# CEED/Laghos

Hardware: AMD Instinct MI355X
Metric: Mdofs×steps/s on 3D Sedov -pa (Q3/Q2) (higher is better)
Workload: dtype f64; 1 GPU; 3D Sedov -p 1 -m cube01_hex -rs 4 -ok 3 -ot 2 -pa (32^3 elements, E0/2^dim = 0.125); transport=none (one rank), elements=32768, h1_dofs=2738019, l2_dofs=884736, quad_points_per_element=216, rk_stages_executed=1300, ode=RK4, parallelism=elements1x1x1, zones_per_gpu=32x32x32

## Files before the change

laghos_amd/csrc/lgh_qpoint.hpp:

```cpp
#pragma once
#include "lgh_common.hpp"
#include "lgh_smallmat.hpp"

namespace lgh
{

enum { QMODE_UPDATE = 0, QMODE_SETUP = 1, QMODE_IE = 2, QMODE_KE = 3 };

struct QArgs
{
   int NE, N;
   const double *B, *G, *Bl, *W;
   const int *map;
   const double *x, *v, *e;
   const double *gamma;
   const double *rho0DetJ0w_in;
   const double *Jac0inv_in;
   const double *Jac0inv_soa;
   const double *Jac0inv_e;
   double *Jac0inv_soa_out;
   double *stressJinvT;
   double *Jac0inv_out, *rho0DetJ0w_out, *massD_out;
   const double *rho0_q;
   double *partials;
   unsigned int *ticket;
   double *result;
   double h0, h1order, cfl;
   int visc, vort;
   double *force_e;
   double *erhs_q;
   int q_swz;
   const int *zorder;
   double tiny_grad;
};

__device__ __forceinline__ double smooth_step_01(double x, double eps)
{
   const double y = (x + eps) / (2.0 * eps);
   if (y < 0.0) { return 0.0; }
   if (y > 1.0) { return 1.0; }
   return (3.0 - 2.0 * y) * y * y;
}

template <int DIM, bool VISC = true>
__device__ __forceinline__ double qpoint_body(const QArgs &a, const int e, const size_t eq,
                                              const double weight, const double *J, const double *dV,
                                              const double e_val, const size_t plane,
                                              const double *J0i, const double rho0DetJ0w, double &ftv, double *sjw)
{
   constexpr int DIM2 = DIM * DIM;
   double Jinv[DIM2], stress[DIM2], sgrad_v[DIM2], stressJiT[DIM2];
   const double gamma = a.gamma[e];
   const double inv_weight = 1. / weight;
   const double detJ = sm::det<DIM>(J);
   sm::inverse<DIM>(J, detJ, Jinv);
   const double R = inv_weight * rho0DetJ0w / detJ;
   const double E = fmax(0.0, e_val);
   const double P = (gamma - 1.0) * R * E;
   const double S = sm::fsqrt(gamma * (gamma - 1.0) * E);
#pragma unroll
   for (int k = 0; k < DIM2; k++) { stress[k] = 0.0; }
#pragma unroll
   for (int d = 0; d < DIM; d++) { stress[d * DIM + d] = -P; }
   double visc_coeff = 0.0;
   double s_dot_g;
   if (VISC && a.visc)
   {
      sm::matmul<DIM>(dV, Jinv, sgrad_v);
      double vorticity_coeff = 1.0;
      if (a.vort)
      {
         const double grad_norm = sm::fnorm<DIM>(sgrad_v);
         const double div_v = fabs(sm::trace<DIM>(sgrad_v));
         vorticity_coeff = (grad_norm > 0.0) ? div_v / grad_norm : 1.0;
      }
      sm::symmetrize<DIM>(sgrad_v);
      double mu, compr_dir[DIM], Jpi[DIM2], ph_dir[DIM];
      bool shortcut = false;
      if (DIM == 3 && a.tiny_grad >= 0.0)
      {
         double m = 0.0;
#pragma unroll
         for (int k = 0; k < DIM2; k++) { m = fmax(m, fabs(sgrad_v[k])); }
         shortcut = __all(m <= a.tiny_grad ? 1 : 0) != 0;
      }
      if (shortcut)
      {
         mu = sm::trace<DIM>(sgrad_v) / 3;
#pragma unroll
         for (int d = 0; d < DIM; d++) { compr_dir[d] = (d == 0) ? 1.0 : 0.0; }
      }
      else { sm::min_eigenpair<DIM>(sgrad_v, mu, compr_dir); }
      sm::matvec<DIM>(J0i, compr_dir, Jpi);
      sm::matvec<DIM>(J, Jpi, ph_dir);
      const double ph_dir_nl2 = sm::norml2<DIM>(ph_dir);
      const double compr_dir_nl2 = sm::norml2<DIM>(compr_dir);
      const double H = a.h0 * ph_dir_nl2 / compr_dir_nl2;
      visc_coeff = 2.0 * R * H * H * fabs(mu);
      const double eps = 1e-12;
      visc_coeff += 0.5 * R * H * S * vorticity_coeff * (1.0 - smooth_step_01(mu - 2.0 * eps, eps));
#pragma unroll
      for (int k = 0; k < DIM2; k++) { stress[k] += visc_coeff * sgrad_v[k]; }
      s_dot_g = 0.0;
#pragma unroll
      for (int k = 0; k < DIM2; k++) { s_dot_g += stress[k] * sgrad_v[k]; }
   }
   else
   {
      double divv = 0.0;
#pragma unroll
      for (int i = 0; i < DIM; i++)
#pragma unroll
         for (int d = 0; d < DIM; d++) { divv += dV[i + DIM * d] * Jinv[d + DIM * i]; }
      s_dot_g = -P * divv;
   }
   const double sv = sm::min_singular<DIM>(J);
   const double h_min = sv / a.h1order;
   const double ih_min = 1. / h_min;
   const double irho_ih_min_sq = ih_min * ih_min / R;
   const double idt = S * ih_min + 2.5 * visc_coeff * irho_ih_min_sq;
   double dt_cand = INFINITY;
   if (detJ < 0.0) { dt_cand = 0.0; }
   else if (idt > 0.0) { dt_cand = a.cfl / idt; }
   sm::matmul_abt<DIM>(stress, Jinv, stressJiT);
   const double wd = weight * detJ;
   ftv = s_dot_g * wd;
#pragma unroll
   for (int vd = 0; vd < DIM; vd++)
#pragma unroll
      for (int gd = 0; gd < DIM; gd++)
      {
         const double sv_ = stressJiT[vd + gd * DIM] * wd;
         sjw[gd + vd * DIM] = sv_;
         if (a.stressJinvT) { a.stressJinvT[eq + plane * (gd + vd * DIM)] = sv_; }
      }
   return dt_cand;
}

template <int DIM, int D, int Q, int L, int NEB, int NFMAX, int MODE, int PPT = 1>
__global__ void __launch_bounds__((DIM == 3 ? Q * Q * Q : Q * Q) * NEB / PPT)
qpoint_kernel(const QArgs a)
{
   constexpr int ND = (DIM == 3) ? D * D * D : D * D;
   constexpr int NQ = (DIM == 3) ? Q * Q * Q : Q * Q;
   constexpr int NL = (DIM == 3) ? L * L * L : L * L;
   constexpr int NTE = NQ / PPT;
   static_assert(PPT == 1 || (PPT == 2 && DIM == 3 && MODE == QMODE_UPDATE && Q % 2 == 0), "two points per thread: 3D update only");
   constexpr bool HOIST = (NQ * NEB <= 256) && PPT == 1;
   constexpr bool NEED_X = (MODE == QMODE_UPDATE || MODE == QMODE_SETUP);
   constexpr bool NEED_V = (MODE == QMODE_UPDATE || MODE == QMODE_KE);
   constexpr bool NEED_E = (MODE != QMODE_KE);
   constexpr int NFIELD = (NEED_X ? DIM : 0) + (NEED_V ? DIM : 0);
   constexpr int NF = (NFIELD == 0) ? 1 : (NFMAX < NFIELD ? NFMAX : NFIELD);
   static_assert(PPT == 1 || NF == NFIELD, "two points per thread: all fields in one LDS pass");
   constexpr int SU = NF * ND;
   constexpr int SXs = (DIM == 3) ? 2 * NF * D * D * Q : 2 * NF * D * Q;
   constexpr int SYs = (DIM == 3) ? 3 * NF * D * Q * Q : 0;
   constexpr int SEs = NL + ((DIM == 3) ? (L * L * Q + L * Q * Q) : (L * Q));
   constexpr int PER0 = SU + SXs + SYs + SEs + 1;
   constexpr int FTN = NQ + ((DIM == 3) ? L * Q * Q : 0);
   constexpr int FNEED3 = 9 * NQ + 9 * D * Q * Q + FTN, FNEED1 = 3 * NQ + 3 * D * Q * Q + FTN;
   constexpr int AVAIL = SU + SXs + SYs + ((DIM == 3) ? L * L * L : L * L);
   constexpr int CPR = (DIM == 3 && MODE == QMODE_UPDATE) ? ((AVAIL >= FNEED3) ? 3 : 1) : 0;
   constexpr int GROW = (CPR == 1 && AVAIL < FNEED1) ? FNEED1 - AVAIL : 0;
   constexpr int PER = PER0 + GROW;
   __shared__ double smem[NEB * PER];
   __shared__ double sB[Q * D], sG[Q * D], sBl[Q * L];
   __shared__ double red[16];

   const int tid = threadIdx.x;
   const int lt = tid % NTE, eb = tid / NTE;
   const int tx = lt % Q, ty = (lt / Q) % Q, tz = lt / (Q * Q);
   const int e = blockIdx.x * NEB + eb;
   const bool active = (e < a.NE);
   const int ec = active ? e : a.NE - 1;
   double *sU = smem + eb * PER;
   double *sX = sU + SU;
   double *sY = sX + SXs;
   double *sE = sY + SYs + GROW;
   double *sE1 = sE + NL;
   double *sE2 = sE1 + ((DIM == 3) ? L * L * Q : 0);

   const size_t eq = (size_t)ec * NQ + lt;

   for (int i = tid; i < Q * D; i += NTE * NEB) { sB[i] = a.B[i]; sG[i] = a.G[i]; }
   for (int i = tid; i < Q * L; i += NTE * NEB) { sBl[i] = a.Bl[i]; }
// ... 631 lines not shown
```

laghos_amd/csrc/lgh_qrows.hpp:

```cpp
#pragma once
#include "lgh_qpoint.hpp"

namespace lgh
{

template <int D, int Q, int L> struct QRows
{
   static constexpr int ND = D * D * D, NQ = Q * Q * Q, NL = L * L * L, NF = 6;
   static constexpr int SU = NF * ND;
   static constexpr int SX = NF * Q * D * D;
   static constexpr int SFS = 9 * NQ + NQ;
   static constexpr int R1 = (SU + 2 * SX > SFS) ? SU + 2 * SX : SFS;
   static constexpr int SY = 3 * NF * Q * Q * D;
   static constexpr int SE = NL + L * L * Q + L * Q * Q;
   static constexpr int ST = 2 * Q * D + Q * L;
   static constexpr int TOTAL = R1 + SY + SE + ST;
};

template <int NIN, int NOUT>
__device__ __forceinline__ void row_fwd(const double *__restrict__ T, const double (&in)[NIN], double (&out)[NOUT])
{
#pragma unroll
   for (int q = 0; q < NOUT; q++)
   {
      double s = T[q * NIN] * in[0];
#pragma unroll
      for (int d = 1; d < NIN; d++) { s = fma(T[q * NIN + d], in[d], s); }
      out[q] = s;
   }
}
template <int NIN, int NOUT>
__device__ __forceinline__ void row_bwd(const double *__restrict__ T, const double (&in)[NIN], double (&out)[NOUT])
{
#pragma unroll
   for (int d = 0; d < NOUT; d++)
   {
      double s = T[d] * in[0];
#pragma unroll
      for (int q = 1; q < NIN; q++) { s = fma(T[q * NOUT + d], in[q], s); }
      out[d] = s;
   }
}
template <int N> __device__ __forceinline__ void row_load(const double *__restrict__ p, double (&v)[N])
{
#pragma unroll
   for (int i = 0; i < N; i++) { v[i] = p[i]; }
}

constexpr int kQTraceRec = 16;
template <int D, int Q, int L, int MINW, bool TRACE = false, bool J0C = false>
__global__ void __launch_bounds__(Q *Q *Q, MINW)
qrows_kernel(const QArgs a, unsigned long long *trace = nullptr)
{
   unsigned long long tstamp[12];
#define LGH_QSTAMP(K_) do { if (TRACE) { tstamp[K_] = wall_clock64(); } } while (0)
   LGH_QSTAMP(0);
   using S = QRows<D, Q, L>;
   constexpr int ND = S::ND, NQ = S::NQ, NL = S::NL, NF = S::NF, NT = NQ;
   constexpr int DD = D * D, QQ = Q * Q;
   __shared__ __attribute__((aligned(16))) double smem[S::TOTAL];
   double *const sR1 = smem;
   double *const sU = sR1;
   double *const sX = sR1 + S::SU;
   double *const sF = sR1;
   double *const sS = sR1 + 9 * NQ;
   double *const sW = sR1;
   double *const sY = smem + S::R1;
   double *const sA = sY;
   double *const sTB = sY + S::SY;
   double *const sTG = sTB + Q * D;
   double *const sTL = sTG + Q * D;
   double *const sE = sTL + Q * L;
   double *const sE1 = sE + NL;
   double *const sE2 = sE1 + L * L * Q;

   const int lt = threadIdx.x;
   const int tx = lt % Q, ty = (lt / Q) % Q, tz = lt / QQ;
   int e = blockIdx.x;
   if (a.q_swz < 0) { e = xcd_swizzle(blockIdx.x, gridDim.x); }
   else if (a.q_swz > 0)
   {
      const int R = 1 << a.q_swz, span = 8 * R, b = blockIdx.x;
      if (b < (int)(gridDim.x / span) * span) { e = (b / span) * span + (b & 7) * R + ((b >> 3) & (R - 1)); }
   }
   if (a.zorder) { e = __builtin_amdgcn_readfirstlane(a.zorder[min(e, a.NE - 1)]); }
   const size_t eq = (size_t)e * NQ + lt;
   const size_t plane = (size_t)a.NE * NQ;

   for (int i = lt; i < Q * D; i += NT)
   {
      const int q = i / D, d = i - q * D;
      sTB[i] = a.B[q + Q * d];
      sTG[i] = a.G[q + Q * d];
   }
   for (int i = lt; i < Q * L; i += NT)
   {
      const int q = i / L, l = i - q * L;
      sTL[i] = a.Bl[q + Q * l];
   }
   for (int i = lt; i < 3 * ND; i += NT)
   {
      const int c = i / ND, d = i - c * ND;
      const size_t n = (size_t)c * a.N + a.map[(size_t)e * ND + d];
      sU[i] = a.x[n];
      sU[i + 3 * ND] = a.v[n];
   }
   for (int i = lt; i < NL; i += NT) { sE[i] = a.e[(size_t)e * NL + i]; }
   double J0i[9];
   if (J0C)
   {
#pragma unroll
      for (int k = 0; k < 9; k++) { J0i[k] = uniform_f64(a.Jac0inv_e[(size_t)9 * e + k]); }
   }
   else
   {
#pragma unroll
      for (int k = 0; k < 9; k++) { J0i[k] = a.Jac0inv_soa[eq + plane * k]; }
   }
   const double rdw = a.rho0DetJ0w_in[eq];
   const double weight = a.W[lt];
   LGH_QSTAMP(1);
   __syncthreads();
   LGH_QSTAMP(2);

   for (int i = lt; i < 2 * NF * DD; i += NT)
   {
      const int which = i / (NF * DD), r = i - which * (NF * DD);
      const double *T = sTB + which * (Q * D);
      double u[D], o[Q];
      row_load<D>(sU + D * r, u);
      row_fwd<D, Q>(T, u, o);
      const int f = r / DD, zy = r - f * DD;
      double *dst = sX + which * S::SX + f * (Q * DD) + zy;
#pragma unroll
      for (int q = 0; q < Q; q++) { dst[q * DD] = o[q]; }
   }
   {
      const int j = NT - 1 - lt;
      if (j < L * L)
      {
         double u[L], o[Q];
         row_load<L>(sE + L * j, u);
         row_fwd<L, Q>(sTL, u, o);
#pragma unroll
         for (int q = 0; q < Q; q++) { sE1[j * Q + q] = o[q]; }
      }
   }
   __syncthreads();
   LGH_QSTAMP(3);

   for (int i = lt; i < 3 * NF * Q * D; i += NT)
   {
      const int part = i / (NF * Q * D), r = i - part * (NF * Q * D);
      const double *T = sTB + ((part == 1) ? Q * D : 0);
      double u[D], o[Q];
      row_load<D>(sX + (part == 0 ? S::SX : 0) + D * r, u);
      row_fwd<D, Q>(T, u, o);
      const int f = r / (Q * D), xz = r - f * (Q * D);
      double *dst = sY + (part * NF + f) * (QQ * D) + xz;
#pragma unroll
      for (int q = 0; q < Q; q++) { dst[q * (Q * D)] = o[q]; }
   }
   {
      const int j = NT - 1 - lt;
      if (j < L * Q)
      {
         const int qx = j % Q, lz = j / Q;
         double u[L], o[Q];
#pragma unroll
         for (int ly = 0; ly < L; ly++) { u[ly] = sE1[(lz * L + ly) * Q + qx]; }
         row_fwd<L, Q>(sTL, u, o);
#pragma unroll
         for (int q = 0; q < Q; q++) { sE2[(lz * Q + q) * Q + qx] = o[q]; }
      }
   }
   __syncthreads();
   LGH_QSTAMP(4);

   double J[9], dV[9], e_val = 0.0;
   {
      double tb[D], tg[D];
      row_load<D>(sTB + D * tz, tb);
      row_load<D>(sTG + D * tz, tg);
      const double *col = sY + (ty * Q + tx) * D;
#pragma unroll
      for (int f = 0; f < NF; f++)
      {
         double gb[D], bg[D], bb[D];
         row_load<D>(col + (0 * NF + f) * (QQ * D), gb);
         row_load<D>(col + (1 * NF + f) * (QQ * D), bg);
         row_load<D>(col + (2 * NF + f) * (QQ * D), bb);
         double d0 = tb[0] * gb[0], d1 = tb[0] * bg[0], d2 = tg[0] * bb[0];
#pragma unroll
         for (int dz = 1; dz < D; dz++)
         {
            d0 = fma(tb[dz], gb[dz], d0);
            d1 = fma(tb[dz], bg[dz], d1);
            d2 = fma(tg[dz], bb[dz], d2);
         }
         double *M = (f < 3) ? J : dV;
         const int c = (f < 3) ? f : f - 3;
         M[c] = d0;
         M[c + 3] = d1;
         M[c + 6] = d2;
      }
#pragma unroll
      for (int lz = 0; lz < L; lz++) { e_val = fma(sTL[tz * L + lz], sE2[(lz * Q + ty) * Q + tx], e_val); }
   }
   LGH_QSTAMP(5);
   double ftv = 0.0, sjw[9];
   const double cand = qpoint_body<3>(a, e, eq, weight, J, dV, e_val, plane, J0i, rdw, ftv, sjw);
   LGH_QSTAMP(6);
   tstamp[7] = tstamp[8] = tstamp[9] = tstamp[10] = 0;

   const bool do_f = (a.force_e != nullptr), do_t = (a.erhs_q != nullptr);
   if (do_f || do_t)
   {
      const int pq = (ty * Q + tx) * Q + tz;
      if (do_f)
      {
#pragma unroll
         for (int k = 0; k < 9; k++) { sF[k * NQ + pq] = sjw[k]; }
      }
      if (do_t) { sS[pq] = ftv; }
      __syncthreads();
      LGH_QSTAMP(7);

      if (do_f)
      {
         for (int i = lt; i < 9 * QQ; i += NT)
         {
            const int k = i / QQ, r = i - k * QQ;
            const double *T = sTB + (((k % 3) == 2) ? Q * D : 0);
            double u[Q], o[D];
            row_load<Q>(sF + (size_t)i * Q, u);
            row_bwd<Q, D>(T, u, o);
            const int qx = r % Q, qy = r / Q;
            double *dst = sA + k * (D * QQ) + qx * Q + qy;
#pragma unroll
            for (int d = 0; d < D; d++) { dst[d * QQ] = o[d]; }
         }
      }
      if (do_t)
      {
         const int j = NT - 1 - lt;
         if (j < QQ)
         {
            double u[Q], o[L];
            row_load<Q>(sS + j * Q, u);
            row_bwd<Q, L>(sTL, u, o);
#pragma unroll
            for (int l = 0; l < L; l++) { sE2[l * QQ + j] = o[l]; }
         }
      }
      __syncthreads();
      LGH_QSTAMP(8);

      if (do_f)
// ... 159 lines not shown
```

laghos_amd/csrc/lgh_qupdate.hip:

```cpp
#include "lgh_qpoint.hpp"
#include "lgh_qrows.hpp"

namespace lgh
{

int qupdate_form(lgh_ctx *c);
int qupdate(lgh_ctx *c, const double *S)
{
   QArgs a = q_base(c);
   a.x = S;
   a.v = S + c->H1V;
   a.e = S + 2 * (size_t)c->H1V;
   a.result = c->dt_est_dev;
   a.Jac0inv_e = (c->jac0_compact == 1) ? c->Jac0inv_e : nullptr;
   const bool keep = !c->stress_store && a.erhs_q && a.force_e && c->v_snap;
   if (keep) { a.stressJinvT = nullptr; }
   const int form = qupdate_form(c);
   const int rc = (form == 1) ? launch_qrows(c, a) : launch_q<QMODE_UPDATE>(c, a);
   c->qgen++;
   c->stress_current = (rc == LGH_OK && !keep) ? 1 : 0;
   c->fused_ftv_valid = (rc == LGH_OK && a.erhs_q && c->v_snap) ? 1 : 0;
   c->fused_f1_valid = (rc == LGH_OK && a.force_e) ? 1 : 0;
   if (c->fused_ftv_valid)
   {
      LGH_HIP_CHECK(hipMemcpyAsync(c->v_snap, S + c->H1V, sizeof(double) * (size_t)c->H1V, hipMemcpyDeviceToDevice, c->stream));
   }
   return rc;
}

int qupdate_form(lgh_ctx *c)
{
   const char *fenv = getenv("LGH_Q_FORM");
   return (qrows_available(c) && !(fenv && fenv[0] == '0')) ? 1 : 0;
}

int interp_energy(lgh_ctx *c, int which, const double *vec, double *result)
{
   QArgs a = q_base(c);
   a.result = c->scal;
   int rc;
   if (which == 0)
   {
      a.e = vec;
      rc = launch_q<QMODE_IE>(c, a);
   }
   else
   {
      a.v = vec;
      rc = launch_q<QMODE_KE>(c, a);
   }
   if (rc) { return rc; }
   if (c->multi != 0)
   {
      rc = allreduce_dev(c, c->scal, 1, 0);
      if (rc) { return rc; }
   }
   LGH_HIP_CHECK(hipMemcpyAsync(c->host_pinned, c->scal, sizeof(double), hipMemcpyDeviceToHost, c->stream));
   LGH_HIP_CHECK(hipStreamSynchronize(c->stream));
   *result = (which == 0) ? c->host_pinned[0] : 0.5 * c->host_pinned[0];
   return LGH_OK;
}

__global__ void __launch_bounds__(128)
tg_source_2d_k(const int NE, const int N, const int D, const int Q, const int L, const int *__restrict__ map,
               const double *__restrict__ B, const double *__restrict__ G, const double *__restrict__ Bl,
               const double *__restrict__ W, const double *__restrict__ x, double *__restrict__ out)
{
   __shared__ double sx[2 * 36], ss[100];
   const int e = blockIdx.x, t = threadIdx.x;
   const int ND = D * D, NQ = Q * Q, NL = L * L;
   for (int i = t; i < 2 * ND; i += blockDim.x)
   {
      const int c = i / ND, d = i - c * ND;
      sx[i] = x[(size_t)c * N + map[(size_t)e * ND + d]];
   }
   __syncthreads();
   if (t < NQ)
   {
      const int qx = t % Q, qy = t / Q;
      double v[2] = {0.0, 0.0}, gx[2] = {0.0, 0.0}, gy[2] = {0.0, 0.0};
      for (int dy = 0; dy < D; dy++)
      {
         for (int dx = 0; dx < D; dx++)
         {
            const double bb = B[qx + Q * dx] * B[qy + Q * dy];
            const double gb = G[qx + Q * dx] * B[qy + Q * dy];
            const double bg = B[qx + Q * dx] * G[qy + Q * dy];
            for (int c = 0; c < 2; c++)
            {
               const double u = sx[c * ND + dx + D * dy];
               v[c] += bb * u;
               gx[c] += gb * u;
               gy[c] += bg * u;
            }
         }
      }
      const double det = gx[0] * gy[1] - gx[1] * gy[0];
      const double f = 3.0 / 8.0 * M_PI * (cos(3.0 * M_PI * v[0]) * cos(M_PI * v[1]) - cos(M_PI * v[0]) * cos(3.0 * M_PI * v[1]));
      ss[t] = W[t] * det * f;
   }
   __syncthreads();
   if (t < NL)
   {
      const int lx = t % L, ly = t / L;
      double s = 0.0;
      for (int qy = 0; qy < Q; qy++)
      {
         for (int qx = 0; qx < Q; qx++) { s += ss[qx + Q * qy] * Bl[qx + Q * lx] * Bl[qy + Q * ly]; }
      }
      out[t + (size_t)NL * e] = s;
   }
}
int tg_source_2d(lgh_ctx *c, const double *S, double *out)
{
   if (c->dim != 2) { set_error("the Taylor-Green energy source is the 2D one (laghos_solver.cpp:448)"); return LGH_ERR_ARG; }
   if (c->D1D > 6 || c->Q1D > 10 || c->NQ > 128) { return LGH_ERR_UNSUPPORTED; }
   hipLaunchKernelGGL(tg_source_2d_k, dim3(c->NE), dim3(128), 0, c->stream, c->NE, c->N, c->D1D, c->Q1D, c->L1D,
                      c->h1map, c->B, c->G, c->Bl, c->W, S, out);
   LGH_HIP_CHECK(hipGetLastError());
   return LGH_OK;
}

template <int DIM>
__global__ void test_eig_k(int n, const double *A, double *lambda, double *vec)
{
   const int i = blockIdx.x * blockDim.x + threadIdx.x;
   if (i >= n) { return; }
   double a[DIM * DIM], v[DIM], l;
   for (int k = 0; k < DIM * DIM; k++) { a[k] = A[(size_t)i * DIM * DIM + k]; }
   sm::min_eigenpair<DIM>(a, l, v);
   lambda[i] = l;
   for (int k = 0; k < DIM; k++) { vec[(size_t)i * DIM + k] = v[k]; }
}
template <int DIM>
__global__ void test_sv_k(int n, const double *A, double *sv)
{
   const int i = blockIdx.x * blockDim.x + threadIdx.x;
   if (i >= n) { return; }
   double a[DIM * DIM];
   for (int k = 0; k < DIM * DIM; k++) { a[k] = A[(size_t)i * DIM * DIM + k]; }
   sv[i] = sm::min_singular<DIM>(a);
}
__global__ void test_sqrt_k(int n, const double *x, double *y)
{
   const int i = blockIdx.x * blockDim.x + threadIdx.x;
   if (i < n) { y[i] = sm::fsqrt(x[i]); }
}
int test_sqrt(lgh_ctx *c, int n, const double *x, double *y)
{
   hipLaunchKernelGGL(test_sqrt_k, dim3(ceil_div(n, 256)), dim3(256), 0, c->stream, n, x, y);
   LGH_HIP_CHECK(hipGetLastError());
   return LGH_OK;
}
int test_eig(lgh_ctx *c, int dim, int n, const double *A, double *lambda, double *vec)
{
   if (dim == 2) { hipLaunchKernelGGL(test_eig_k<2>, dim3(ceil_div(n, 128)), dim3(128), 0, c->stream, n, A, lambda, vec); }
   else { hipLaunchKernelGGL(test_eig_k<3>, dim3(ceil_div(n, 128)), dim3(128), 0, c->stream, n, A, lambda, vec); }
   LGH_HIP_CHECK(hipGetLastError());
   return LGH_OK;
}
int test_singular(lgh_ctx *c, int dim, int n, const double *A, double *sv)
{
   if (dim == 2) { hipLaunchKernelGGL(test_sv_k<2>, dim3(ceil_div(n, 128)), dim3(128), 0, c->stream, n, A, sv); }
   else { hipLaunchKernelGGL(test_sv_k<3>, dim3(ceil_div(n, 128)), dim3(128), 0, c->stream, n, A, sv); }
   LGH_HIP_CHECK(hipGetLastError());
   return LGH_OK;
}

}
```

laghos_amd/csrc/lgh_vcg.hip:

```cpp
#include "lgh_vcg.hpp"

namespace lgh
{
typedef unsigned v4u_ __attribute__((ext_vector_type(4)));


template <int D, int Q, int NEB>
__global__ void __launch_bounds__(Q *Q *NEB, (Q >= 8) ? 1 : 2)
vcg_apply_3d(const VcgArgs a, const int nbatch)
{
   constexpr int NQ = Q * Q * Q, ND = D * D * D;
   constexpr int SX = (ND > D * Q * Q) ? ND : D * Q * Q;
   constexpr int SA = D * D * Q;
   constexpr int SAE = (SA > D * Q * D) ? SA : D * Q * D;
   constexpr int OFF_A = kVC * SX, OFF_IN = OFF_A + kVC * SAE;
   constexpr int PER = OFF_IN + kVC * ND + 1;
   constexpr int NT = Q * Q * NEB;
   constexpr int GPT = (NEB * ND + NT - 1) / NT;
   __shared__ double smem[NEB * PER];
   __shared__ double red[48];

   if (a.s->all_done) { return; }
   const int tid = threadIdx.x;
   const int tx = tid % Q, ty = (tid / Q) % Q, eb = tid / (Q * Q);
// ... 787 lines not shown
         part = fma(sIn[base + DD * i], v, part);
      }
      dot[0] += (k2 == 0) ? part : 0.0;
      dot[1] += (k2 == 1) ? part : 0.0;
      dot[2] += (k2 == 2) ? part : 0.0;
   }
   double bp[kVC];
   block_sum3(dot[0], dot[1], dot[2], red, bp);
   double total[kVC];
   if (grid_sum3_last_block(bp, a.partials, a.stride, a.ticket, red, total))
   {
      if (tid == 0)
      {
         VcgScalars *s = a.s;
         for (int k = 0; k < kVC; k++)
         {
            if (!todo[k]) { continue; }
            s->den[k] = total[k];
            if (total[k] == 0.0 && !a.multi) { s->done[k] = 1; }
         }
         s->first = 0;
      }
   }
}

__device__ __forceinline__ double vcg_ld(const double *base, const unsigned off) { return *(const double *)((const char *)base + off); }
__device__ __forceinline__ double *vcg_ptr(double *base, const unsigned off) { return (double *)((char *)base + off); }

__device__ __forceinline__ void vcg_reset_accumulators(const VcgArgs &a)
{
   if (!a.reset || blockIdx.x != 0) { return; }
   if (a.limbs) { for (int i = threadIdx.x; i < 2 * kLimbWords + 8 * 16; i += blockDim.x) { a.limbs[i] = 0; } }
   if (a.rzl) { for (int i = threadIdx.x; i < 3 * kLimbWords; i += blockDim.x) { a.rzl[i] = 0; } }
}
__device__ __forceinline__ void vcg_reset_scalars(const VcgArgs &a, VcgScalars *s)
{
   if (!a.reset) { return; }
   s->rel_tol2 = a.reset_tol2;
   s->all_done = 0;
   s->first = 1;
   for (int c = 0; c < kVC; c++) { s->done[c] = 0; s->iters[c] = 0; s->nupd[c] = 0; s->alpha_last[c] = 0.0; s->alpha_hist[0][c] = s->alpha_hist[1][c] = 0.0; s->rzh[0][c] = s->rzh[1][c] = 0.0; }
}

__global__ void __launch_bounds__(256)
vcg_init_k(const VcgArgs a)
{
   vcg_reset_accumulators(a);
   __shared__ double red[48];
   const int n = xcd_swizzle(blockIdx.x, gridDim.x) * blockDim.x + threadIdx.x;
   double part[kVC] = {0.0, 0.0, 0.0};
   if (n < a.N)
   {
      const double di = a.dinv[n];
      const double ow = a.owner ? a.owner[n] : 1.0;
#pragma unroll
      for (int c = 0; c < kVC; c++)
      {
         const size_t i = (size_t)c * a.N + n;
         const double rv = a.b[(size_t)c * a.N + (a.ncaller ? a.ncaller[n] : n)];
         a.r[i] = rv;
         part[c] = ow * __dmul_rn(rv, di) * rv;
      }
   }
   double bp[kVC], total[kVC];
   block_sum3(part[0], part[1], part[2], red, bp);
   if (grid_sum3_last_block(bp, a.partials, a.stride, a.ticket, red, total))
   {
      if (threadIdx.x == 0)
      {
         VcgScalars *s = a.s;
         int all = 1;
         vcg_reset_scalars(a, s);
         for (int c = 0; c < kVC; c++)
         {
            s->rz[c] = s->rz_prev[c] = total[c];
            s->iters[c] = 0;
            if (!a.multi)
            {
               s->r0[c] = fmax(total[c] * s->rel_tol2, 0.0);
               s->done[c] = (total[c] < 0.0 || total[c] <= s->r0[c]) ? 1 : 0;
               all = all && s->done[c];
            }
         }
         s->first = 1;
         if (!a.multi) { s->all_done = all; }
      }
   }
}
template <int DEG>
__global__ void __launch_bounds__(256)
vcg_init_force_k(const VcgArgs a, const double *__restrict__ FE, const int ND, double *__restrict__ bout, const int *__restrict__ ellc, const int degc)
{
   vcg_reset_accumulators(a);
   __shared__ double red[48];
   const int n = xcd_swizzle(blockIdx.x, gridDim.x) * blockDim.x + threadIdx.x;
   double part[kVC] = {0.0, 0.0, 0.0};
   if (n < a.N)
   {
      long pos[DEG];
#pragma unroll
      for (int j = 0; j < DEG; j++)
      {
         const int p = (j < degc) ? ellc[(size_t)j * a.N + n] : -1;
         const int e = p / ND;
         pos[j] = (p >= 0) ? (long)kVC * ND * e + (p - e * ND) : -1;
      }
      const double di = a.dinv[n];
#pragma unroll
      for (int c = 0; c < kVC; c++)
      {
         double s = 0.0;
#pragma unroll
         for (int j = 0; j < DEG; j++) { if (pos[j] >= 0) { s += FE[pos[j] + (long)ND * c]; } }
         double bv = -s;
         if (a.ess[c] && a.ess[c][n]) { bv = 0.0; }
         const size_t i = (size_t)c * a.N + n;
         bout[(size_t)c * a.N + (a.ncaller ? a.ncaller[n] : n)] = bv;
         a.r[i] = bv;
         a.x[i] = 0.0;
         part[c] = __dmul_rn(bv, di) * bv;
      }
   }
   double bp[kVC], total[kVC];
   block_sum3(part[0], part[1], part[2], red, bp);
   if (grid_sum3_last_block(bp, a.partials, a.stride, a.ticket, red, total))
   {
      if (threadIdx.x == 0)
      {
         VcgScalars *s = a.s;
         int all = 1;
         vcg_reset_scalars(a, s);
         for (int c = 0; c < kVC; c++)
         {
            s->rz[c] = s->rz_prev[c] = total[c];
            s->iters[c] = 0;
            s->r0[c] = fmax(total[c] * s->rel_tol2, 0.0);
            s->done[c] = (total[c] < 0.0 || total[c] <= s->r0[c]) ? 1 : 0;
            all = all && s->done[c];
         }
         s->first = 1;
         s->all_done = all;
      }
   }
}
__global__ void __launch_bounds__(256)
vcg_init_force_z_k(const VcgArgs a, const double *__restrict__ FE, const unsigned compb_fe, const unsigned *__restrict__ ellf,
                   double *__restrict__ bout)
{
   vcg_reset_accumulators(a);
   __shared__ double red[48];
   const int n = xcd_swizzle(blockIdx.x, gridDim.x) * blockDim.x + threadIdx.x;
   const bool ok = n < a.N;
   const unsigned nn = (unsigned)(ok ? n : a.N - 1);
   const unsigned rowb = 4u * (unsigned)a.N;
   unsigned ix[8];
#pragma unroll
   for (int j = 0; j < 8; j++) { ix[j] = *(const unsigned *)((const char *)ellf + (4u * nn + (unsigned)j * rowb)); }
   const double di = vcg_ld(a.dinv, 8u * nn);
   const unsigned es = a.essbits[nn];
   const unsigned zoff = 8u * (unsigned)kVC * (unsigned)(a.ye_stride - kYePad);
   double fe[kVC][8];
#pragma unroll
   for (int j = 0; j < 8; j++)
   {
      if (j == 0 || __any(ix[j] != zoff))
      {
#pragma unroll
         for (int c = 0; c < kVC; c++) { fe[c][j] = vcg_ld(FE, ix[j] + (unsigned)c * compb_fe); }
      }
      else
      {
#pragma unroll
         for (int c = 0; c < kVC; c++) { fe[c][j] = 0.0; }
      }
   }
   double part[kVC];
#pragma unroll
   for (int c = 0; c < kVC; c++)
   {
      double s = 0.0;
#pragma unroll
      for (int j = 0; j < 8; j++) { s += fe[c][j]; }
      double bv = -s;
      if ((es >> c) & 1u) { bv = 0.0; }
      part[c] = ok ? __dmul_rn(bv, di) * bv : 0.0;
      if (ok)
      {
         const size_t i = (size_t)c * a.N + n;
         bout[(size_t)c * a.N + (a.ncaller ? a.ncaller[n] : n)] = bv;
         a.r[i] = bv;
         a.x[i] = 0.0;
      }
   }
   double bp[kVC], total[kVC];
   block_sum3(part[0], part[1], part[2], red, bp);
   if (grid_sum3_last_block(bp, a.partials, a.stride, a.ticket, red, total))
   {
      if (threadIdx.x == 0)
      {
         VcgScalars *s = a.s;
         int all = 1;
         vcg_reset_scalars(a, s);
         for (int c = 0; c < kVC; c++)
         {
            s->rz[c] = s->rz_prev[c] = total[c];
            s->iters[c] = 0;
            s->r0[c] = fmax(total[c] * s->rel_tol2, 0.0);
            s->done[c] = (total[c] < 0.0 || total[c] <= s->r0[c]) ? 1 : 0;
            all = all && s->done[c];
         }
         s->first = 1;
         s->all_done = all;
      }
   }
}
__global__ void __launch_bounds__(256)
vcg_ellf_k(const int *__restrict__ ell, unsigned *__restrict__ ellf, const size_t n_have, const size_t n_all, const int ND, const int NE)
{
   const size_t i = (size_t)blockIdx.x * blockDim.x + threadIdx.x;
   if (i >= n_all) { return; }
   const int p = (i < n_have) ? ell[i] : -1;
   const int e = p / ND;
   ellf[i] = 8u * (unsigned)(p < 0 ? kVC * ND * NE : kVC * ND * e + (p - e * ND));
}
__global__ void __launch_bounds__(256)
vcg_mapb_k(const int *__restrict__ map, unsigned *__restrict__ mapb, const size_t n)
{
   const size_t i = (size_t)blockIdx.x * blockDim.x + threadIdx.x;
   if (i < n) { mapb[i] = 8u * (unsigned)map[i]; }
}
__global__ void __launch_bounds__(256)
vcg_map_xrows_k(const int *__restrict__ map, const size_t nrows, const int D, int *flag)
{
   const size_t i = (size_t)blockIdx.x * blockDim.x + threadIdx.x;
   if (i >= nrows) { return; }
   const int *p = map + i * D;
   bool ok = true;
   for (int k = 1; k < D; k++) { ok = ok && p[k] == p[0] + k; }
   if (!ok) { *flag = 1; }
}
__global__ void vcg_init_finish_k(VcgScalars *s)
{
   int all = 1;
   for (int c = 0; c < kVC; c++)
   {
      s->rz_prev[c] = s->rz[c];
      s->r0[c] = fmax(s->rz[c] * s->rel_tol2, 0.0);
      s->done[c] = (s->rz[c] < 0.0 || s->rz[c] <= s->r0[c]) ? 1 : 0;
      all = all && s->done[c];
   }
   s->all_done = all;
}
__global__ void vcg_set_tol_k(VcgScalars *s, double rel_tol2, long long *limbs, long long *rzl)
{
   if (limbs) { for (int i = 0; i < 2 * kLimbWords + 8 * 16; i++) { limbs[i] = 0; } }
   if (rzl) { for (int i = 0; i < 3 * kLimbWords; i++) { rzl[i] = 0; } }
   s->rel_tol2 = rel_tol2;
   s->all_done = 0;
   s->first = 1;
   for (int c = 0; c < kVC; c++) { s->done[c] = 0; s->iters[c] = 0; s->nupd[c] = 0; s->alpha_last[c] = 0.0; s->alpha_hist[0][c] = s->alpha_hist[1][c] = 0.0; s->rzh[0][c] = s->rzh[1][c] = 0.0; }
}
__global__ void vcg_update_finish_k(VcgScalars *s, int iter, VcgScalars *host_out, unsigned long long *host_token, const unsigned long long token)
{
   int all = 1;
   for (int c = 0; c < kVC; c++)
   {
      if (!s->done[c])
      {
         s->iters[c] = iter;
         if (s->rz[c] < 0.0 || s->rz[c] <= s->r0[c]) { s->done[c] = 1; }
      }
      if (s->done[c]) { s->rz[c] = 0.0; s->den[c] = 0.0; }
      all = all && s->done[c];
   }
   s->all_done = all;
   if (host_out)
   {
      *host_out = *s;
      __threadfence_system();
      __hip_atomic_store(host_token, token, __ATOMIC_RELEASE, __HIP_MEMORY_SCOPE_SYSTEM);
   }
}

__global__ void vcg_rz_finish_k(VcgScalars *s, const long long *rzl, const int last, const long long *peers, const int n_peers, VcgScalars *host_out,
                                unsigned long long *host_token, const unsigned long long token)
{
   long long set[kLimbWords];
   for (int i = 0; i <= kLimbShards * kVC * kLimbs; i++)
   {
      long long w = rzl[(last % 3) * kLimbWords + i];
      for (int p = 0; p < n_peers; p++) { w += peers[p * kLimbWords + i]; }
      set[i] = w;
   }
   double cur[kVC];
   bool dn[kVC];
   for (int k = 0; k < kVC; k++)
   {
      const double before = (last > 1) ? s->rzh[(last - 1) & 1][k] : s->rz[k];
      cur[k] = exact_fold(set, k, exact_scale(before));
      dn[k] = s->done[k] != 0 || vcg_rz_converged(last + 1, cur[k], s->r0[k]);
   }
   vcg_rz_commit(s, last + 1, cur, dn);
   if (host_out)
   {
      *host_out = *s;
      __threadfence_system();
      __hip_atomic_store(host_token, token, __ATOMIC_RELEASE, __HIP_MEMORY_SCOPE_SYSTEM);
   }
}

template <bool FUSED_GATHER, int DEG>
__global__ void __launch_bounds__(256)
vcg_update_k(const VcgArgs a)
{
   __shared__ double red[48];
   if (a.s->all_done) { return; }
   const bool it1 = (a.iter == 1);
   const int n = xcd_swizzle(blockIdx.x, gridDim.x) * blockDim.x + threadIdx.x;
   const bool ok = n < a.N;
   const int nn = ok ? n : a.N - 1;
   double part[kVC] = {0.0, 0.0, 0.0};
   int pidx[DEG > 0 ? DEG : 1];
   if (FUSED_GATHER)
   {
#pragma unroll
      for (int j = 0; j < DEG; j++) { pidx[j] = (j < a.deg) ? a.ell[(size_t)j * a.N + nn] : -1; }
   }
   const double di = a.dinv[nn];
   const double ow = a.owner ? a.owner[nn] : 1.0;
   const bool shared = FUSED_GATHER && a.hmask && a.hmask[nn];
#pragma unroll 1
   for (int c = 0; c < kVC; c++)
   {
      if (a.s->done[c]) { continue; }
      if (a.multi && vcg_pending_den(a.s, c, blockIdx.x == 0 && threadIdx.x == 0)) { continue; }
      const double alpha = a.s->rz[c] / a.s->den[c];
      const double beta = it1 ? 0.0 : a.s->rz[c] / a.s->rz_prev[c];
      const size_t i = (size_t)c * a.N + nn;
      double zv;
      if (FUSED_GATHER)
      {
         if (shared) { zv = a.yL[i]; }
         else
         {
            const double *yc = a.YE + (size_t)c * a.ye_stride;
            zv = 0.0;
#pragma unroll
            for (int j = 0; j < DEG; j++) { if (pidx[j] >= 0) { zv += yc[pidx[j]]; } }
         }
      }
      else { zv = a.yL[i]; }
      if (a.ess[c] && a.ess[c][nn]) { zv = 0.0; }
      const double ro = a.r[i];
      double dv = __dmul_rn(ro, di);
      if (!it1) { dv = fma(beta, a.d[i], dv); }
      const double xv = a.x[i] + alpha * dv;
      const double rv = ro - alpha * zv;
      const double pz = __dmul_rn(rv, di);
      if (ok)
      {
         a.d[i] = dv;
         a.x[i] = xv;
         a.r[i] = rv;
         part[c] = ow * rv * pz;
      }
   }
   double bp[kVC], total[kVC];
   block_sum3(part[0], part[1], part[2], red, bp);
   if (grid_sum3_last_block(bp, a.partials, a.stride, a.ticket, red, total))
   {
      if (threadIdx.x == 0)
      {
         VcgScalars *s = a.s;
         int all = 1;
         for (int c = 0; c < kVC; c++)
         {
// ... 1624 lines not shown
```

Measured before the change: 1578 Mdofs*steps/s.

## Fuse velocity snapshot into qrows gather and repack ELL force indices as uint4

The quadrature-row kernel now writes the velocity snapshot while gathering nodal velocities, which removes the separate full device-to-device copy after the update. The ELL force-gather index table is repacked so each node's first four and last four indices sit in contiguous 16-byte groups, loaded with vector loads. The second half is only fetched when some lane in the wavefront has a valid fourth entry. The fused snapshot writes each shared node once per element that touches it (redundant, but the same value), and the index layout change depends on N being n_all/8.

```diff
diff --git a/laghos_amd/csrc/lgh_qpoint.hpp b/laghos_amd/csrc/lgh_qpoint.hpp
--- a/laghos_amd/csrc/lgh_qpoint.hpp
+++ b/laghos_amd/csrc/lgh_qpoint.hpp
@@ -32,6 +32,7 @@
    int q_swz;
    const int *zorder;
    double tiny_grad;
+   double *v_snap;
 };
 
 __device__ __forceinline__ double smooth_step_01(double x, double eps)
diff --git a/laghos_amd/csrc/lgh_qrows.hpp b/laghos_amd/csrc/lgh_qrows.hpp
--- a/laghos_amd/csrc/lgh_qrows.hpp
+++ b/laghos_amd/csrc/lgh_qrows.hpp
@@ -102,8 +102,10 @@
    {
       const int c = i / ND, d = i - c * ND;
       const size_t n = (size_t)c * a.N + a.map[(size_t)e * ND + d];
+      const double vn = a.v[n];
+      if (a.v_snap) { a.v_snap[n] = vn; }
       sU[i] = a.x[n];
-      sU[i + 3 * ND] = a.v[n];
+      sU[i + 3 * ND] = vn;
    }
    for (int i = lt; i < NL; i += NT) { sE[i] = a.e[(size_t)e * NL + i]; }
    double J0i[9];
diff --git a/laghos_amd/csrc/lgh_qupdate.hip b/laghos_amd/csrc/lgh_qupdate.hip
--- a/laghos_amd/csrc/lgh_qupdate.hip
+++ b/laghos_amd/csrc/lgh_qupdate.hip
@@ -16,12 +16,14 @@
    const bool keep = !c->stress_store && a.erhs_q && a.force_e && c->v_snap;
    if (keep) { a.stressJinvT = nullptr; }
    const int form = qupdate_form(c);
+   const bool snap = a.erhs_q && c->v_snap;
+   if (form == 1 && snap) { a.v_snap = c->v_snap; }
    const int rc = (form == 1) ? launch_qrows(c, a) : launch_q<QMODE_UPDATE>(c, a);
    c->qgen++;
    c->stress_current = (rc == LGH_OK && !keep) ? 1 : 0;
-   c->fused_ftv_valid = (rc == LGH_OK && a.erhs_q && c->v_snap) ? 1 : 0;
+   c->fused_ftv_valid = (rc == LGH_OK && snap) ? 1 : 0;
    c->fused_f1_valid = (rc == LGH_OK && a.force_e) ? 1 : 0;
-   if (c->fused_ftv_valid)
+   if (c->fused_ftv_valid && !a.v_snap)
    {
       LGH_HIP_CHECK(hipMemcpyAsync(c->v_snap, S + c->H1V, sizeof(double) * (size_t)c->H1V, hipMemcpyDeviceToDevice, c->stream));
    }
diff --git a/laghos_amd/csrc/lgh_vcg.hip b/laghos_amd/csrc/lgh_vcg.hip
--- a/laghos_amd/csrc/lgh_vcg.hip
+++ b/laghos_amd/csrc/lgh_vcg.hip
@@ -963,42 +963,67 @@
    const int n = xcd_swizzle(blockIdx.x, gridDim.x) * blockDim.x + threadIdx.x;
    const bool ok = n < a.N;
    const unsigned nn = (unsigned)(ok ? n : a.N - 1);
-   const unsigned rowb = 4u * (unsigned)a.N;
-   unsigned ix[8];
-#pragma unroll
-   for (int j = 0; j < 8; j++) { ix[j] = *(const unsigned *)((const char *)ellf + (4u * nn + (unsigned)j * rowb)); }
+   const unsigned zoff = 8u * (unsigned)kVC * (unsigned)(a.ye_stride - kYePad);
+   const v4u_ q0 = *(const v4u_ *)((const char *)ellf + 16u * nn);
    const double di = vcg_ld(a.dinv, 8u * nn);
    const unsigned es = a.essbits[nn];
-   const unsigned zoff = 8u * (unsigned)kVC * (unsigned)(a.ye_stride - kYePad);
-   double fe[kVC][8];
-#pragma unroll
-   for (int j = 0; j < 8; j++)
-   {
-      if (j == 0 || __any(ix[j] != zoff))
+   const unsigned nc = a.ncaller ? (unsigned)a.ncaller[nn] : nn;
+   const unsigned ix[4] = {q0[0], q0[1], q0[2], q0[3]};
+   double s[kVC];
+   if (__any(ix[3] != zoff))
+   {
+      const v4u_ q1 = *(const v4u_ *)((const char *)ellf + (size_t)16 * (size_t)a.N + 16u * nn);
+      double fe[kVC][8];
+#pragma unroll
+      for (int j = 0; j < 4; j++)
       {
 #pragma unroll
          for (int c = 0; c < kVC; c++) { fe[c][j] = vcg_ld(FE, ix[j] + (unsigned)c * compb_fe); }
       }
-      else
-      {
-#pragma unroll
-         for (int c = 0; c < kVC; c++) { fe[c][j] = 0.0; }
-      }
+#pragma unroll
+      for (int j = 0; j < 4; j++)
+      {
+#pragma unroll
+         for (int c = 0; c < kVC; c++) { fe[c][4 + j] = vcg_ld(FE, q1[j] + (unsigned)c * compb_fe); }
+      }
+#pragma unroll
+      for (int c = 0; c < kVC; c++)
+      {
+         s[c] = (((0.0 + fe[c][0]) + fe[c][1]) + fe[c][2]) + fe[c][3];
+         s[c] = (((s[c] + fe[c][4]) + fe[c][5]) + fe[c][6]) + fe[c][7];
+      }
+   }
+   else
+   {
+      double fe[kVC][3];
+#pragma unroll
+      for (int j = 0; j < 3; j++)
+      {
+         if (j == 0 || __any(ix[j] != zoff))
+         {
+#pragma unroll
+            for (int c = 0; c < kVC; c++) { fe[c][j] = vcg_ld(FE, ix[j] + (unsigned)c * compb_fe); }
+         }
+         else
+         {
+#pragma unroll
+            for (int c = 0; c < kVC; c++) { fe[c][j] = 0.0; }
+         }
+      }
+#pragma unroll
+      for (int c = 0; c < kVC; c++) { s[c] = ((0.0 + fe[c][0]) + fe[c][1]) + fe[c][2]; }
    }
    double part[kVC];
 #pragma unroll
    for (int c = 0; c < kVC; c++)
    {
-      double s = 0.0;
-#pragma unroll
-      for (int j = 0; j < 8; j++) { s += fe[c][j]; }
-      double bv = -s;
+      double bv = -s[c];
       if ((es >> c) & 1u) { bv = 0.0; }
       part[c] = ok ? __dmul_rn(bv, di) * bv : 0.0;
       if (ok)
       {
          const size_t i = (size_t)c * a.N + n;
-         bout[(size_t)c * a.N + (a.ncaller ? a.ncaller[n] : n)] = bv;
+         bout[(size_t)c * a.N + nc] = bv;
          a.r[i] = bv;
          a.x[i] = 0.0;
       }
@@ -1009,19 +1034,19 @@
    {
       if (threadIdx.x == 0)
       {
-         VcgScalars *s = a.s;
+         VcgScalars *s_ = a.s;
          int all = 1;
-         vcg_reset_scalars(a, s);
+         vcg_reset_scalars(a, s_);
          for (int c = 0; c < kVC; c++)
          {
-            s->rz[c] = s->rz_prev[c] = total[c];
-            s->iters[c] = 0;
-            s->r0[c] = fmax(total[c] * s->rel_tol2, 0.0);
-            s->done[c] = (total[c] < 0.0 || total[c] <= s->r0[c]) ? 1 : 0;
-            all = all && s->done[c];
-         }
-         s->first = 1;
-         s->all_done = all;
+            s_->rz[c] = s_->rz_prev[c] = total[c];
+            s_->iters[c] = 0;
+            s_->r0[c] = fmax(total[c] * s_->rel_tol2, 0.0);
+            s_->done[c] = (total[c] < 0.0 || total[c] <= s_->r0[c]) ? 1 : 0;
+            all = all && s_->done[c];
+         }
+         s_->first = 1;
+         s_->all_done = all;
       }
    }
 }
@@ -1032,7 +1057,8 @@
    if (i >= n_all) { return; }
    const int p = (i < n_have) ? ell[i] : -1;
    const int e = p / ND;
-   ellf[i] = 8u * (unsigned)(p < 0 ? kVC * ND * NE : kVC * ND * e + (p - e * ND));
+   const size_t N = n_all / 8, j = i / N, n = i - j * N;
+   ellf[(j < 4 ? 0 : 4 * N) + 4 * n + (j & 3)] = 8u * (unsigned)(p < 0 ? kVC * ND * NE : kVC * ND * e + (p - e * ND));
 }
 __global__ void __launch_bounds__(256)
 vcg_mapb_k(const int *__restrict__ map, unsigned *__restrict__ mapb, const size_t n)
```

After: 1578 Mdofs*steps/s. About the same (-0.0%).
